# mozendr/FHE-SPEAR

Hardware: AMD Instinct MI355X
Metric: BSGS matvecs/sec at d=2048,N=16384,L0=36; sec/RWKV-block at 1/2/4/8 GPU (higher is better)
Workload: dtype u64

## Files before the change

fhe-spear_amd/csrc/fhs_kernels.hip:

```cpp
#include "fhs_kernels.h"
typedef unsigned long long u64x2_t __attribute__((ext_vector_type(2)));
#ifndef FHS_MODUP_STORE_AUX
#define FHS_MODUP_STORE_AUX 2
#endif
#ifndef FHS_KSIP_UNROLL
#define FHS_KSIP_UNROLL 4
#endif
#include "fhs_ntt.h"
#include "fhs_buffer.h"

#include <atomic>
#include <cstdio>
#include <cstdlib>
#include <cstring>
#include <vector>
#include <algorithm>

#define FHS_INNER_WAVES 16
#define FHS_INNER_VEC 2
#ifndef FHS_MODUPH_CH
#define FHS_MODUPH_CH 2
#endif
#ifndef FHS_MODUPH_RL
#define FHS_MODUPH_RL 3
// ... 1488 lines not shown
                          const KTimer* tm, unsigned* zflag = nullptr) {
    FHS_TMARK(tm, KID_KS_INTT, 1, st);
    if (ks_intt_half<LOGN>(l * U))
        hipLaunchKernelGGL((k_ks_intt_h<LOGN>), dim3(l * U), dim3((1 << LOGN) / 32), 0, st, T, uniq, b.acoef, l, U);
    else
        hipLaunchKernelGGL((k_ks_intt<LOGN>), dim3(l * U), dim3((1 << LOGN) / 16), 0, st, T, uniq, b.acoef, l, U);
    launch_centered(T, b.acoef, b.vcnt, l, U, st, zflag);
    FHS_TMARK(tm, KID_KS_INTT, 0, st);
}
template <int LOGN>
static void ks_modup_stage(const DevTables& T, const u64* const* uniq, int U, int l, const KsBufs& b, hipStream_t st,
                           const KTimer* tm) {
    FHS_TMARK(tm, KID_MODUP, 1, st);
    launch_modup<LOGN>(T, uniq, b.acoef, b.vcnt, b.ext, l, U, st);
    FHS_TMARK(tm, KID_MODUP, 0, st);
}
static void ks_ip_stage(const DevTables& T, const KsItem* it, const u64* const* uniq, int R, int l, const KsBufs& b,
                        hipStream_t st, const KTimer* tm) {
    FHS_TMARK(tm, KID_KS_IP, 1, st);
    hipLaunchKernelGGL(k_ks_ip, dim3(xcd_grid(l + T.P, R * (T.N >> 8))), dim3(256), 0, st, T, it, uniq, b.ext, b.acc, l, R,
                       0);
    FHS_TMARK(tm, KID_KS_IP, 0, st);
}
static void giant_ip_stage(const DevTables& T, const KsItem* it, const u64* const* uniq, int R, int l, const KsBufs& b,
                           hipStream_t st, const KTimer* tm) {
    const int NB = T.N >> 8;
    FHS_TMARK(tm, KID_KS_IP, 1, st);
    hipLaunchKernelGGL(k_ks_ip, dim3(T.P * R * NB), dim3(256), 0, st, T, it, uniq, b.ext, b.acc, l, R, l);
    hipLaunchKernelGGL(k_ks_ip_sum, dim3(xcd_grid(l, NB)), dim3(256), 0, st, T, it, uniq, b.ext, b.acc, l, R);
    FHS_TMARK(tm, KID_KS_IP, 0, st);
}
template <int LOGN>
static void ks_special_intt_stage(const DevTables& T, int R, int l, const KsBufs& b, hipStream_t st, const KTimer* tm) {
    FHS_TMARK(tm, KID_SPECIAL_INTT, 1, st);
    FHS_NTT_LAUNCH(k_ks_special_intt, T.P * 2 * R, dim3(T.P, 2, R), st, T, b.acc, b.ycoef, l, R);
    FHS_TMARK(tm, KID_SPECIAL_INTT, 0, st);
}
template <int LOGN>
static hipError_t ks_moddown_stage(const DevTables& T, const KsItem* it, int R, int l, const KsBufs& b, hipStream_t st,
                                   const KTimer* tm) {
    FHS_TMARK(tm, KID_MODDOWN, 1, st);
    void (*k)(DevTables, const KsItem*, const u64*, const u64*, int, int);
    int nwg = l * 2 * R, threads = (1 << LOGN) / 32;
    const bool xform = ks_uses_half(LOGN) && T.md_xform;
    if (!ks_uses_half(LOGN)) {
        k = k_moddown<LOGN>;
        threads = (1 << LOGN) / 16;
    } else if (xform && T.conv_b59 && LOGN == 15 && nwg < FHS_SPLIT_MAX_WG) {
        k = k_moddown_h<LOGN, true, true, true>;
        nwg *= 2;
    } else if (xform) {
        k = T.conv_b59 ? k_moddown_h<LOGN, true, true> : k_moddown_h<LOGN, true>;
    } else {
        k = T.all_b59 ? k_moddown_h<LOGN, false, true> : k_moddown_h<LOGN, false>;
    }
    if (xform)
        hipLaunchKernelGGL(k_special_x, dim3((T.N + 255) / 256, 2 * R), dim3(256), 0, st, T, b.ycoef, 2 * R);
    hipLaunchKernelGGL(k, dim3(nwg), dim3(threads), 0, st, T, it, b.acc, b.ycoef, l, R);
    FHS_TMARK(tm, KID_MODDOWN, 0, st);
    return hipGetLastError();
}

static hipError_t upload_items(const KsItem* items, int R, const u64* const* uniq, int U, void* dev, const Stager& sg,
                               const KsItem** it_dev, const u64* const** uniq_dev) {
    static thread_local std::vector<unsigned char> buf;
    buf.resize(sizeof(KsItem) * R + sizeof(u64*) * U);
    memcpy(buf.data(), items, sizeof(KsItem) * R);
    memcpy(buf.data() + sizeof(KsItem) * R, uniq, sizeof(u64*) * U);
    hipError_t e = sg.h2d(sg.user, dev, buf.data(), buf.size());
    *it_dev = reinterpret_cast<const KsItem*>(dev);
    *uniq_dev = reinterpret_cast<const u64* const*>(static_cast<unsigned char*>(dev) + sizeof(KsItem) * R);
    return e;
}

__global__ void k_seal_mask(DevTables T, u64 elt, u64* out) {
    const int N = T.N, i = blockIdx.x * blockDim.x + threadIdx.x;
    if (i >= N) return;
    const u64 j = ((u64)i * elt) & (2 * (u64)N - 1);
    const u64 v = j >> T.logN;
    const size_t k = j & (N - 1);
    for (int t = 0; t < T.K; ++t) out[(size_t)t * N + k] = v;
}
__global__ void __launch_bounds__(256) k_seal_corr(DevTables T, const u64* key, const u64* akey, const u64* M,
                                                    int l, u64* out) {
    const int N = T.N, K = T.K, E = l + T.P;
    const int n = blockIdx.x * blockDim.x + threadIdx.x, t = blockIdx.y;
    if (n >= N || t >= E) return;
    const int pt = t < l ? t : T.L0 + (t - l);
    const RedU RD = redu(PK(T, pt));
    const u64 p = RD.q;
    const unsigned qb = 64 - __clzll(p);
    const u64* seeds = key + (size_t)T.dnum * K * N;
    const u64 cx = seeded_ctr_mix(pt, n);
    u128 s0 = {0, 0}, s1 = {0, 0};
    for (int j = 0; j < l; ++j) {
        if (j == t) continue;
        const u64 qj = reduce128(PK(T, j).q, 0, RD);
        const size_t kx = ((size_t)j * K + pt) * N + n;
        const u64 a = akey ? akey[kx] : seeded_uniform_x(seeds[j] + cx, p, qb);
        mac128(s0, key[kx], qj);
        mac128(s1, a, qj);
        if ((j & 7) == 7) {
            s0 = u128{reduce128(s0.lo, s0.hi, RD), 0};
            s1 = u128{reduce128(s1.lo, s1.hi, RD), 0};
        }
    }
    const u64 m = M[(size_t)pt * N + n];
    const u64 r0 = reduce128(s0.lo, s0.hi, RD), r1 = reduce128(s1.lo, s1.hi, RD);
    out[(size_t)t * N + n] = reduce128(r0 * m, __umul64hi(r0, m), RD);
    out[((size_t)E + t) * N + n] = reduce128(r1 * m, __umul64hi(r1, m), RD);
}
hipError_t launch_seal_corr(const DevTables& T, const u64* key, const u64* akey, u64 elt, int l, u64* mask_scratch,
                            u64* out, hipStream_t st) {
    if (T.P != 1 || l < 1 || l > T.L0 || !key || !out || !mask_scratch) return hipErrorInvalidValue;
    hipLaunchKernelGGL(k_seal_mask, dim3((T.N + 255) / 256), dim3(256), 0, st, T, elt, mask_scratch);
    hipError_t e = launch_ntt_fwd(T, mask_scratch, T.K, T.L0, 1, 0, st);
    if (e != hipSuccess) return e;
    hipLaunchKernelGGL(k_seal_corr, dim3((T.N + 255) / 256, l + T.P), dim3(256), 0, st, T, key, akey, mask_scratch,
                       l, out);
    return hipGetLastError();
}

hipError_t launch_keyswitch(const DevTables& T, const KsItem* items_host, int R, const u64* const* uniq_host, int U,
                            int l, u64* ws, size_t ws_bytes, void* items_dev, const Stager& sg, hipStream_t st,
                            const KTimer* tm, SealHoist* sh) {
    if (keyswitch_workspace_bytes(T, R, U, l) > ws_bytes) return hipErrorInvalidValue;
    const KsItem* it;
    const u64* const* uq;
    std::vector<KsItem> sitems;
    std::vector<const u64*> suniq;
    bool hoist = T.ks_seal && sh && U < R;
    for (int r = 0; hoist && r < R; ++r) hoist = items_host[r].elt == 1 || items_host[r].corr;
    if (hoist) {
        hipError_t e = upload_items(items_host, R, uniq_host, U, items_dev, sg, &it, &uq);
        if (e == hipSuccess) e = hipMemsetAsync(sh->zflag_dev, 0, sizeof(unsigned), st);
        if (e != hipSuccess) return e;
        const KsBufs b = ks_carve(T, ws, R, U, l);
        FHS_DISPATCH_LOGN(T.logN, ks_intt_stage<LOGN>(T, uq, U, l, b, st, tm, sh->zflag_dev));
        e = hipMemcpyAsync(sh->zflag_host, sh->zflag_dev, sizeof(unsigned), hipMemcpyDeviceToHost, st);
        if (e == hipSuccess) e = hipStreamSynchronize(st);
        if (e != hipSuccess) return e;
        if (*(volatile unsigned*)sh->zflag_host) {
            ++sh->fallback;
            return launch_keyswitch(T, items_host, R, uniq_host, U, l, ws, ws_bytes, items_dev, sg, st, tm, nullptr);
        }
        ++sh->hoisted;
        FHS_DISPATCH_LOGN(T.logN, {
            ks_modup_stage<LOGN>(T, uq, U, l, b, st, tm);
            ks_ip_stage(T, it, uq, R, l, b, st, tm);
            ks_special_intt_stage<LOGN>(T, R, l, b, st, tm);
            e = ks_moddown_stage<LOGN>(T, it, R, l, b, st, tm);
        });
        if (e != hipSuccess) return e;
        return hipGetLastError();
    }
    if (T.ks_seal) {
        sitems.assign(items_host, items_host + R);
        suniq.resize(R);
        u64* perm = ws + ks_core_bytes(T, R, R, l) / 8;
        seal_rewrite(T, sitems.data(), R, suniq.data(), l, perm);
        hipError_t pe = seal_permute(T, items_host, R, l, perm, st);
        if (pe != hipSuccess) return pe;
        items_host = sitems.data();
        uniq_host = suniq.data();
        U = R;
    }
    hipError_t e = upload_items(items_host, R, uniq_host, U, items_dev, sg, &it, &uq);
    if (e != hipSuccess) return e;
    hipError_t me = hipSuccess;
    const KsBufs b = ks_carve(T, ws, R, U, l);
    FHS_DISPATCH_LOGN(T.logN, {
        ks_intt_stage<LOGN>(T, uq, U, l, b, st, tm);
        ks_modup_stage<LOGN>(T, uq, U, l, b, st, tm);
        ks_ip_stage(T, it, uq, R, l, b, st, tm);
        ks_special_intt_stage<LOGN>(T, R, l, b, st, tm);
        me = ks_moddown_stage<LOGN>(T, it, R, l, b, st, tm);
    });
    if (me != hipSuccess) return me;
    return hipGetLastError();
}

template <int VEC, int TL = 0>
__device__ __forceinline__ void ld_diag(const u64* limb, int voff, int soff, u64* out) {
    const __amdgpu_buffer_rsrc_t r = brsrc(limb, 0x7ffffff0);
    if constexpr (TL > 0) {
        static_assert(VEC == 2, "compact diagonals: two coefficients per lane");
        out[0] = out[1] = __builtin_bit_cast(u64, __builtin_amdgcn_raw_buffer_load_b64(r, voff, soff, kBufNT));
    } else if constexpr (VEC == 2) {
        const auto t = __builtin_amdgcn_raw_buffer_load_b128(r, voff, soff, kBufNT);
        out[0] = ((u64)t[1] << 32) | t[0];
        out[1] = ((u64)t[3] << 32) | t[2];
    } else {
        out[0] = __builtin_bit_cast(u64, __builtin_amdgcn_raw_buffer_load_b64(r, voff, soff, kBufNT));
    }
}
template <int VEC, int WAVES, int FOLD, bool ACC, int TL = 0>
__global__ void __launch_bounds__(64 * WAVES) k_bsgs_inner(DevTables T, const u64* const* __restrict__ baby,
                                                    const u64* const* __restrict__ pts, int G, int Gw, int g0, int g1,
                                                    int D, int l, u64* __restrict__ inner) {
    extern __shared__ __attribute__((aligned(16))) u64 sb[];
    constexpr int W = 64 * VEC;
    const int N = T.N;
    const int i = blockIdx.y, n0 = blockIdx.x * W, tid = threadIdx.x, lane = tid & 63;
    const int wave = __builtin_amdgcn_readfirstlane(tid >> 6);
    const size_t S = (size_t)l * N;
    const size_t off = (size_t)i * N + n0 + lane * VEC;
    const size_t dlimb = (size_t)i * (N >> TL);
    const int dvoff = ((lane * VEC) >> TL) * 8, dsoff = (n0 >> TL) * 8;
    u64 p[8][VEC];
    const int gcur = g0 + wave;
    auto full_batches = [&](int g) { return g < g1 ? max(0, min(Gw, D - g * G)) / 8 : 0; };
    int gf = gcur;
    while (gf < g1 && full_batches(gf) == 0) gf += WAVES;
    if (gf < g1) {
        const u64* const* pg0 = pts + (size_t)gf * G;
#pragma unroll
        for (int u = 0; u < 8; ++u) ld_diag<VEC, TL>(pg0[u] + dlimb, dvoff, dsoff, p[u]);
    }
    for (int idx = tid; idx < Gw * 2 * W; idx += 64 * WAVES) {
        const int b = idx / (2 * W), comp = (idx / W) & 1, c = idx % W;
        sb[idx] = pack30(baby[b][comp * S + (size_t)i * N + n0 + c]);
    }
    __syncthreads();
    const RedU R = redu(PK(T, i));
    for (int g = gcur; g < g1; g += WAVES) {
        const int bmax = min(Gw, D - g * G);
        if (bmax <= 0) continue;
        u128 c0[VEC], c1[VEC];
        Acc3 a0[VEC], a1[VEC];
#pragma unroll
        for (int v = 0; v < VEC; ++v) {
            c0[v] = c1[v] = u128{0, 0};
            a0[v] = a1[v] = Acc3{0, 0, 0};
        }
        const u64* const* pg = pts + (size_t)g * G;
        const int nb = bmax / 8;
        int gn = g + WAVES;
        while (gn < g1 && full_batches(gn) == 0) gn += WAVES;
        int b = 0;
        for (int bi = 0; bi < nb; ++bi, b += 8) {
            constexpr bool ROLL = FOLD == 16;
            if (!ROLL && bi > 0) {
#pragma unroll
                for (int u = 0; u < 8; ++u) ld_diag<VEC, TL>(pg[b + u] + dlimb, dvoff, dsoff, p[u]);
            }
            const u64* const* nxt = ROLL && bi + 1 < nb ? pg + b + 8 : nullptr;
#pragma unroll
            for (int h = 0; h < 8; h += 4) {
#pragma unroll
                for (int u = h; u < h + 4; ++u)
#pragma unroll
                    for (int v = 0; v < VEC; ++v) {
                        const Split30 y = split30(p[u][v]);
                        acc3_mac(a0[v], unpack30(sb[((b + u) * 2 + 0) * W + lane * VEC + v]), y);
                        acc3_mac(a1[v], unpack30(sb[((b + u) * 2 + 1) * W + lane * VEC + v]), y);
                    }
                if (h == 4 && (FOLD == 8 || (b & 15) == 8)) {
#pragma unroll
                    for (int v = 0; v < VEC; ++v) {
                        acc3_fold(c0[v], a0[v]);
                        acc3_fold(c1[v], a1[v]);
                    }
                }
                if (nxt) {
#pragma unroll
                    for (int u = h; u < h + 4; ++u) ld_diag<VEC, TL>(nxt[u] + dlimb, dvoff, dsoff, p[u]);
                }
            }
        }
        for (; b < bmax; ++b) {
            u64 q1[VEC];
            ld_diag<VEC, TL>(pg[b] + dlimb, dvoff, dsoff, q1);
#pragma unroll
            for (int v = 0; v < VEC; ++v) {
                const Split30 y = split30(q1[v]);
                acc3_mac(a0[v], unpack30(sb[(b * 2 + 0) * W + lane * VEC + v]), y);
                acc3_mac(a1[v], unpack30(sb[(b * 2 + 1) * W + lane * VEC + v]), y);
            }
        }
#pragma unroll
        for (int v = 0; v < VEC; ++v) {
            acc3_fold(c0[v], a0[v]);
            acc3_fold(c1[v], a1[v]);
        }
#pragma unroll
        for (int v = 0; v < VEC; ++v) {
            u64* o0 = inner + (size_t)g * 2 * S + off + v;
            u64 r0 = reduce128(c0[v].lo, c0[v].hi, R), r1 = reduce128(c1[v].lo, c1[v].hi, R);
            if constexpr (ACC) {
                r0 = addmod(r0, o0[0], R.q);
                r1 = addmod(r1, o0[S], R.q);
            }
            o0[0] = r0;
            o0[S] = r1;
        }
        if (gn < g1) {
            const u64* const* pgn = pts + (size_t)gn * G;
#pragma unroll
            for (int u = 0; u < 8; ++u) ld_diag<VEC, TL>(pgn[u] + dlimb, dvoff, dsoff, p[u]);
        }
    }
}

#ifndef FHS_GSUM_ICH
#define FHS_GSUM_ICH 4
#endif
__global__ void __launch_bounds__(256) k_giant_sum(DevTables T, const u64* bpart, const u64* ycoef, const u64* inner0,
                                                   u64* base, u64* convsum, int l, int R) {
    const int N = T.N, P_ = T.P, E = l + P_;
    const int n = blockIdx.x * blockDim.x + threadIdx.x, comp = blockIdx.y;
    if (n >= N) return;
    const int i0 = blockIdx.z * FHS_GSUM_ICH, i1 = min(i0 + FHS_GSUM_ICH, l);
    const size_t S = (size_t)l * N;
    constexpr int PMAX = 8;
    u64 ylo[PMAX], yhi[PMAX];
#pragma unroll
    for (int k = 0; k < PMAX; ++k) ylo[k] = yhi[k] = 0;
    for (int r = 0; r < R; ++r) {
        const u64* y = ycoef + ((size_t)r * 2 + comp) * P_ * N + n;
#pragma unroll
        for (int k = 0; k < PMAX; ++k) {
            if (k < P_) {
                const u64 v = y[(size_t)k * N];
                ylo[k] += v;
                yhi[k] += ylo[k] < v;
            }
        }
    }
    for (int i = i0; i < i1; ++i) {
        const PrimeK& P = PK(T, i);
        const u64 q = P.q;
        u128 cs = {0, 0};
#pragma unroll
        for (int k = 0; k < PMAX; ++k)
            if (k < P_) mac128(cs, reduce128(ylo[k], yhi[k], P), T.md_hat[(size_t)k * T.L0 + i]);
        if (T.ks_seal) {
            u128 h = {0, 0};
            mac128(h, (u64)R, T.md_pinv[3 * T.L0 + i]);
            const u64 rh = reduce128(h.lo, h.hi, P);
            cs.lo = reduce128(cs.lo, cs.hi, P);
            cs.hi = 0;
            cs.lo = submod(cs.lo, rh, q);
        }
        u64 cv = reduce128(cs.lo, cs.hi, P);
        const size_t idx = (size_t)comp * S + (size_t)i * N + n;
        const u64 bv = addmod(bpart[((size_t)comp * E + i) * N + n], inner0[idx], q);
        convsum[idx] = cv;
        base[idx] = bv;
    }
}
template <int LOGN, bool H = ntt_half<LOGN>()>
__global__ void __launch_bounds__((ntt_threads<LOGN, H>())) k_giant_final(DevTables T, const u64* base, const u64* convsum,
                                                                     u64* out, int l) {
    constexpr int N = 1 << LOGN;
    __shared__ __attribute__((aligned(16))) u64 lds[ntt_lds_words<LOGN, H>()];
    const int i = blockIdx.x, comp = blockIdx.y;
    const PrimeK& P = PK(T, i);
    const RedU RU = redu(P);
    const size_t off = ((size_t)comp * l + i) * N;
    const u64 pinv = T.md_pinv[2 * i], pinv_s = T.md_pinv[2 * i + 1], q = RU.q;
    fwd_limb<LOGN, FHS_NTT_RL, H>(lds, threadIdx.x, T.tw_fwd + (size_t)i * N * 2, RU,
                               [&](int e) { return convsum[off + e]; },
                               [&](int e, u64 v) { out[off + e] = submod(base[off + e], shoup(v, pinv, pinv_s, q), q); });
}

size_t bsgs_workspace_bytes(const DevTables& T, int R, int l) {
    return keyswitch_workspace_bytes(T, R, R, l) + 8 * (size_t)T.N * 4 * l;
}

template <class Each>
static hipError_t lds_opt_in(std::atomic<bool>& done, size_t bytes, Each each) {
    if (done.load(std::memory_order_acquire)) return hipSuccess;
    hipError_t e = hipSuccess;
    each([&](const void* k) {
        if (k && e == hipSuccess) e = hipFuncSetAttribute(k, hipFuncAttributeMaxDynamicSharedMemorySize, (int)bytes);
    });
    if (e == hipSuccess) done.store(true, std::memory_order_release);
    return e;
}

constexpr int kInnerWindow = 64;
typedef void (*InnerFn)(DevTables, const u64* const*, const u64* const*, int, int, int, int, int, int, u64*);
template <int VEC, int WAVES, int FOLD, int TL>
static InnerFn inner_kernel_acc(bool acc) {
    return acc ? k_bsgs_inner<VEC, WAVES, FOLD, true, TL> : k_bsgs_inner<VEC, WAVES, FOLD, false, TL>;
}
template <int VEC, int WAVES>
static InnerFn inner_kernel(bool fold16, bool acc, int ptl) {
    if (!fold16) return ptl == 0 ? inner_kernel_acc<VEC, WAVES, 8, 0>(acc) : nullptr;
    switch (ptl) {
        case 0: return inner_kernel_acc<VEC, WAVES, 16, 0>(acc);
        case 1: return inner_kernel_acc<VEC, WAVES, 16, 1>(acc);
        case 2: return inner_kernel_acc<VEC, WAVES, 16, 2>(acc);
        case 3: return inner_kernel_acc<VEC, WAVES, 16, 3>(acc);
    }
    return nullptr;
}
template <int VEC, int WAVES>
static hipError_t launch_inner_t(const DevTables& T, const u64* const* baby, const u64* const* pts, int G, int g0,
                                 int g1, int D, int l, u64* inner, hipStream_t st, int ptl) {
    constexpr int W = 64 * VEC;
    static std::atomic<bool> opted{false};
    hipError_t e = lds_opt_in(opted, (size_t)kInnerWindow * 2 * W * 8, [](auto f) {
        for (int fold16 = 0; fold16 < 2; ++fold16)
            for (int acc = 0; acc < 2; ++acc)
                for (int tl = 0; tl <= 3; ++tl)
                    f(reinterpret_cast<const void*>(inner_kernel<VEC, WAVES>(fold16, acc, tl)));
    });
    if (e != hipSuccess) return e;
    if (ptl < 0 || ptl > 3 || (ptl > 0 && (T.max_qbits > 59 || VEC != 2))) return hipErrorInvalidValue;
    for (int b0 = 0; b0 < G; b0 += kInnerWindow) {
        const int Gw = std::min(kInnerWindow, G - b0), Dw = D - b0;
        const size_t lds = (size_t)Gw * 2 * W * 8;
        const dim3 grid(T.N / W, l), block(64 * WAVES);
        const InnerFn k = inner_kernel<VEC, WAVES>(T.max_qbits <= 59, b0 > 0, ptl);
        hipLaunchKernelGGL(k, grid, block, lds, st, T, baby + b0, pts + b0, G, Gw, g0, g1, Dw, l, inner);
        e = hipGetLastError();
        if (e != hipSuccess) return e;
    }
    return hipSuccess;
}

hipError_t launch_bsgs_inner(const DevTables& T, const u64* const* baby_dev, const u64* const* pts_dev, int G, int g0,
                             int g1, int D, int l, u64* inner, hipStream_t st, int ptl) {
    if (T.N % 128 || G < 1) return hipErrorInvalidValue;
    return launch_inner_t<FHS_INNER_VEC, FHS_INNER_WAVES>(T, baby_dev, pts_dev, G, g0, g1, D, l, inner, st, ptl);
}

#define FHS_DOT_WAVES 8
#define FHS_DOT_VEC 2
constexpr int kDotBatch = 4;
template <int VEC, int WAVES, int FOLD, bool ACC>
__global__ void __launch_bounds__(64 * WAVES) k_dot_tensor(DevTables T, const u64* const* __restrict__ q,
                                                          const u64* const* __restrict__ db, int J, int Jw, int C, int l,
                                                          u64* __restrict__ out) {
    extern __shared__ __attribute__((aligned(16))) u64 sb[];
    constexpr int W = 64 * VEC;
    const int N = T.N;
    const int i = blockIdx.y, n0 = blockIdx.x * W, tid = threadIdx.x, lane = tid & 63;
    const int wave = __builtin_amdgcn_readfirstlane(tid >> 6);
    const size_t S = (size_t)l * N;
    const size_t limb = (size_t)i * N;
    const int dvoff = lane * VEC * 8, dsoff = n0 * 8;
    u64 p[kDotBatch][2][VEC];
    auto load_term = [&](const u64* ct, u64 (*dst)[VEC]) {
        ld_diag<VEC>(ct + limb, dvoff, dsoff, dst[0]);
        ld_diag<VEC>(ct + S + limb, dvoff, dsoff, dst[1]);
    };
    const int nb = Jw / kDotBatch;
    if (wave < C && nb > 0) {
        const u64* const* d0 = db + (size_t)wave * J;
#pragma unroll
        for (int u = 0; u < kDotBatch; ++u) load_term(d0[u], p[u]);
    }
    for (int idx = tid; idx < Jw * 2 * W; idx += 64 * WAVES) {
        const int j = idx / (2 * W), comp = (idx / W) & 1, c = idx % W;
        sb[idx] = pack30(q[j][comp * S + limb + n0 + c]);
    }
    __syncthreads();
    const RedU R = redu(PK(T, i));
    for (int c = wave; c < C; c += WAVES) {
        Dot3 s[VEC];
#pragma unroll
        for (int v = 0; v < VEC; ++v) dot3_clear(s[v]);
        const u64* const* dc = db + (size_t)c * J;
        int j = 0;
        for (int bi = 0; bi < nb; ++bi, j += kDotBatch) {
            const u64* const* nxt = bi + 1 < nb ? dc + j + kDotBatch : nullptr;
#pragma unroll
            for (int u = 0; u < kDotBatch; ++u) {
#pragma unroll
                for (int v = 0; v < VEC; ++v)
                    dot3_term<FOLD>(s[v], j + u, unpack30(sb[((j + u) * 2 + 0) * W + lane * VEC + v]),
                                    unpack30(sb[((j + u) * 2 + 1) * W + lane * VEC + v]), split30(p[u][0][v]),
                                    split30(p[u][1][v]));
                if (nxt) load_term(nxt[u], p[u]);
            }
        }
        for (; j < Jw; ++j) {
            u64 t[2][VEC];
            load_term(dc[j], t);
#pragma unroll
            for (int v = 0; v < VEC; ++v)
                dot3_term<FOLD>(s[v], j, unpack30(sb[(j * 2 + 0) * W + lane * VEC + v]),
                                unpack30(sb[(j * 2 + 1) * W + lane * VEC + v]), split30(t[0][v]), split30(t[1][v]));
        }
        u64* o = out + (size_t)c * 3 * S + limb + n0 + lane * VEC;
#pragma unroll
        for (int v = 0; v < VEC; ++v) {
            u64 prev[3], r[3];
            if constexpr (ACC) {
                prev[0] = o[v];
                prev[1] = o[S + v];
                prev[2] = o[2 * S + v];
            }
            dot3_finish(s[v], R, ACC ? prev : nullptr, r);
            o[v] = r[0];
            o[S + v] = r[1];
            o[2 * S + v] = r[2];
        }
        if (c + WAVES < C && nb > 0) {
            const u64* const* dn = db + (size_t)(c + WAVES) * J;
#pragma unroll
            for (int u = 0; u < kDotBatch; ++u) load_term(dn[u], p[u]);
        }
    }
}
typedef void (*DotFn)(DevTables, const u64* const*, const u64* const*, int, int, int, int, u64*);
template <int VEC, int WAVES>
static DotFn dot_kernel(bool fold16, bool acc) {
    if (fold16) return acc ? k_dot_tensor<VEC, WAVES, 16, true> : k_dot_tensor<VEC, WAVES, 16, false>;
    return acc ? k_dot_tensor<VEC, WAVES, 8, true> : k_dot_tensor<VEC, WAVES, 8, false>;
}
template <int VEC, int WAVES>
static hipError_t launch_dot_t(const DevTables& T, const u64* const* q, const u64* const* db, int J, int C, int l, u64* out,
                               hipStream_t st) {
    constexpr int W = 64 * VEC;
    static std::atomic<bool> opted{false};
    hipError_t e = lds_opt_in(opted, (size_t)kDotWindowMax * 2 * W * 8, [](auto f) {
        for (int fold16 = 0; fold16 < 2; ++fold16)
            for (int acc = 0; acc < 2; ++acc) f(reinterpret_cast<const void*>(dot_kernel<VEC, WAVES>(fold16, acc)));
    });
    if (e != hipSuccess) return e;
    for (int j0 = 0; j0 < J; j0 += kDotWindowMax) {
        const int Jw = std::min(kDotWindowMax, J - j0);
        const size_t lds = (size_t)Jw * 2 * W * 8;
        const dim3 grid(T.N / W, l), block(64 * WAVES);
        const DotFn k = dot_kernel<VEC, WAVES>(T.max_qbits <= 59, j0 > 0);
        hipLaunchKernelGGL(k, grid, block, lds, st, T, q + j0, db + j0, J, Jw, C, l, out);
        e = hipGetLastError();
        if (e != hipSuccess) return e;
    }
    return hipSuccess;
}
hipError_t launch_dot_tensor(const DevTables& T, const u64* const* q_dev, const u64* const* db_dev, int J, int C, int l,
                             u64* out3, hipStream_t st, const KTimer* tm) {
    if (T.N % (64 * FHS_DOT_VEC) || J < 1 || C < 1) return hipErrorInvalidValue;
    FHS_TMARK(tm, KID_DOT_TENSOR, 1, st);
    const hipError_t e = launch_dot_t<FHS_DOT_VEC, FHS_DOT_WAVES>(T, q_dev, db_dev, J, C, l, out3, st);
    FHS_TMARK(tm, KID_DOT_TENSOR, 0, st);
    return e;
}

hipError_t launch_bsgs(const DevTables& T, const u64* const* baby_dev, const u64* const* pts_dev, int G, int B, int D,
                       int l, const u64* const* keys_host, const u64* const* akeys_host, const u64* giant_elts, u64* inner,
                       u64* out, u64* ws, size_t ws_bytes, void* items_dev, const Stager& sg, hipStream_t st,
                       const KTimer* tm, int ptl) {
    const int R = B - 1;
    const size_t N = T.N, S = (size_t)l * N;
    if (T.N % 128 || G < 1 || R > 512) return hipErrorInvalidValue;
    if (R > 0 && bsgs_workspace_bytes(T, R, l) > ws_bytes) return hipErrorInvalidValue;
    KsItem items[512];
    const u64* uniq[512];
    for (int r = 0; r < R; ++r) {
        const int g = r + 1;
        const u64* ct = inner + (size_t)g * 2 * S;
        u64 elt = 1;
        if (giant_elts) elt = giant_elts[g];
        else
            for (int s2 = 0; s2 < g * G; ++s2) elt = (elt * 5) & (2 * N - 1);
        items[r] = KsItem{ct + S, ct, nullptr, keys_host[g], nullptr, nullptr, elt, (u64)r,
                          akeys_host ? akeys_host[g] : nullptr};
        uniq[r] = ct + S;
    }
    std::vector<KsItem> seal_orig;
    u64* seal_perm = ws + ks_core_bytes(T, R, R, l) / 8;
    if (T.ks_seal && R > 0) {
        seal_orig.assign(items, items + R);
        seal_rewrite(T, items, R, uniq, l, seal_perm);
    }
    const KsItem* it = nullptr;
    const u64* const* uq = nullptr;
    if (R > 0) {
        hipError_t e = upload_items(items, R, uniq, R, items_dev, sg, &it, &uq);
        if (e != hipSuccess) return e;
    }
    hipError_t he = hipSuccess;
    if (pts_dev) {
        FHS_TMARK(tm, KID_BSGS_INNER, 1, st);
        he = launch_inner_t<FHS_INNER_VEC, FHS_INNER_WAVES>(T, baby_dev, pts_dev, G, 0, B, D, l, inner, st, ptl);
        FHS_TMARK(tm, KID_BSGS_INNER, 0, st);
        if (he != hipSuccess) return he;
    }
    if (R <= 0) return hipMemcpyAsync(out, inner, 8 * 2 * S, hipMemcpyDeviceToDevice, st);
    if (!seal_orig.empty()) {
        he = seal_permute(T, seal_orig.data(), R, l, seal_perm, st);
        if (he != hipSuccess) return he;
    }
    u64* base = ws + keyswitch_workspace_bytes(T, R, R, l) / 8;
    u64* convsum = base + 2 * S;
    FHS_DISPATCH_LOGN(T.logN, {
        const KsBufs b = ks_carve(T, ws, R, R, l);
        ks_intt_stage<LOGN>(T, uq, R, l, b, st, tm);
        ks_modup_stage<LOGN>(T, uq, R, l, b, st, tm);
        giant_ip_stage(T, it, uq, R, l, b, st, tm);
        ks_special_intt_stage<LOGN>(T, R, l, b, st, tm);
        FHS_TMARK(tm, KID_GIANT_SUM, 1, st);
        hipLaunchKernelGGL(k_giant_sum, dim3((T.N + 255) / 256, 2, (l + FHS_GSUM_ICH - 1) / FHS_GSUM_ICH), dim3(256), 0,
                           st, T, b.acc, b.ycoef, inner, base, convsum, l, R);
        FHS_TMARK(tm, KID_GIANT_SUM, 0, st);
        FHS_TMARK(tm, KID_GIANT_FINAL, 1, st);
        FHS_NTT_LAUNCH(k_giant_final, l * 2, dim3(l, 2), st, T, base, convsum, out, l);
        FHS_TMARK(tm, KID_GIANT_FINAL, 0, st);
    });
    return hipGetLastError();
}



__device__ __forceinline__ u64 rnd_testdata(u64 key, u64 ctr) { return sm64(key ^ sm64(ctr ^ 0xD1B54A32D192ED03ULL)); }

__global__ void k_sample(DevTables T, int mode, PrfKey K, u64 sid, u64* out, int l, u64 sid_step, u64* const* outs) {
    const int N = T.N;
    const size_t S = (size_t)l * N;
    sid += blockIdx.y * sid_step;
    out = outs ? outs[blockIdx.y] : out + blockIdx.y * S;
    for (size_t idx = blockIdx.x * (size_t)blockDim.x + threadIdx.x; idx < S; idx += (size_t)gridDim.x * blockDim.x) {
        const int i = (int)(idx / N), n = (int)(idx % N);
        const PrimeK& P = PK(T, i);
        u64 v;
        if (mode == SAMPLE_UNIFORM) {
            u64 hi, lo;
            prf128(K, sid, (uint32_t)idx, hi, lo);
            v = reduce128(lo, hi, P);
        } else if (mode == SAMPLE_SEEDED) {
            v = seeded_uniform_x(sid + seeded_ctr_mix(i, n), P.q, 64 - __clzll(P.q));
        } else if (mode == SAMPLE_TESTDATA) {
            const u64 ctr = 2 * ((u64)i * N + n);
            v = reduce128(rnd_testdata(sid, ctr + 1), rnd_testdata(sid, ctr), P);
        } else {
            u64 r, unused;
            prf128(K, sid, (uint32_t)n, r, unused);
            long long s;
            if (mode == SAMPLE_TERNARY) {
                const u64 t = r % 3;
                s = t == 2 ? -1 : (long long)t;
            } else {
                s = (long long)__popcll(r & 0x1FFFFFULL) - (long long)__popcll((r >> 21) & 0x1FFFFFULL);
            }
            v = s >= 0 ? (u64)s : P.q - (u64)(-s);
        }
        out[idx] = v;
    }
}
hipError_t launch_sample(const DevTables& T, int mode, const PrfKey& K, u64 sid, u64* out, int l, hipStream_t st,
                         int npoly, u64 sid_step, u64* const* outs_dev) {
    if (npoly < 1) return hipSuccess;
    const int g1 = eltwise_grid((size_t)l * T.N) / npoly, gx = g1 > 0 ? g1 : 1;
    hipLaunchKernelGGL(k_sample, dim3(gx, npoly), dim3(256), 0, st, T, mode, K, sid, out, l, sid_step, outs_dev);
    return hipGetLastError();
}

__global__ void k_swk(DevTables T, u64* b_out, const u64* a, const u64* e, const u64* s, const u64* snew, int j) {
    const int N = T.N, K = T.K;
    const size_t S = (size_t)K * N;
    for (size_t idx = blockIdx.x * (size_t)blockDim.x + threadIdx.x; idx < S; idx += (size_t)gridDim.x * blockDim.x) {
        const int i = (int)(idx / N);
        const PrimeK& P = PK(T, i);
        u64 v = submod(e[idx], mulmod(a[idx], s[idx], P), P.q);
        if (i < T.L0 && i / T.P == j) {
            const u64 pm = T.md_pinv[2 * T.L0 + i];
            v = addmod(v, mulmod(pm, snew[idx], P), P.q);
        }
        b_out[idx] = v;
    }
}
hipError_t launch_switch_key_assemble(const DevTables& T, u64* b_out, const u64* a, const u64* e_ntt, const u64* s_ntt,
                                      const u64* snew_ntt, int digit, hipStream_t st) {
    hipLaunchKernelGGL(k_swk, dim3(eltwise_grid((size_t)T.K * T.N)), dim3(256), 0, st, T, b_out, a, e_ntt, s_ntt,
                       snew_ntt, digit);
    return hipGetLastError();
}

__global__ void k_encrypt(DevTables T, int mode, u64* c0, u64* c1, const u64* s_or_pk0, const u64* pk1, const u64* u,
                          const u64* e0, const u64* e1, const u64* pt, int l) {
    const int N = T.N;
    const size_t S = (size_t)l * N;
    for (size_t idx = blockIdx.x * (size_t)blockDim.x + threadIdx.x; idx < S; idx += (size_t)gridDim.x * blockDim.x) {
        const int i = (int)(idx / N);
        const PrimeK& P = PK(T, i);
        const u64 q = P.q;
        const u64 m = pt ? pt[idx] : 0;
        if (mode == 0) {
            c0[idx] = addmod(submod(e0[idx], mulmod(c1[idx], s_or_pk0[idx], P), q), m, q);
        } else {
            c0[idx] = addmod(addmod(mulmod(u[idx], s_or_pk0[idx], P), e0[idx], q), m, q);
            c1[idx] = addmod(mulmod(u[idx], pk1[idx], P), e1[idx], q);
        }
    }
}
__global__ void k_sample_small(int mode, PrfKey K, u64 sid, u64 sid_step, int N, signed char* out) {
    sid += blockIdx.y * sid_step;
    out += (size_t)blockIdx.y * N;
    for (int n = blockIdx.x * blockDim.x + threadIdx.x; n < N; n += gridDim.x * blockDim.x) {
        u64 r, unused;
        prf128(K, sid, (uint32_t)n, r, unused);
        int v;
        if (mode == SAMPLE_TERNARY) {
            const u64 t = r % 3;
            v = t == 2 ? -1 : (int)t;
        } else {
            v = __popcll(r & 0x1FFFFFULL) - __popcll((r >> 21) & 0x1FFFFFULL);
        }
        out[n] = (signed char)v;
    }
}
template <int LOGN>
__global__ void __launch_bounds__(ntt_threads<LOGN>()) k_ntt_fwd_small(DevTables T, const signed char* small, u64* out,
                                                                      int limbs) {
    constexpr int N = 1 << LOGN;
    __shared__ __attribute__((aligned(16))) u64 lds[ntt_lds_words<LOGN>()];
    const int b = blockIdx.x;
    const RedU R = redu(PK(T, b));
    const signed char* sm = small + (size_t)blockIdx.y * N;
    u64* p = out + ((size_t)blockIdx.y * limbs + b) * N;
    const u64 q = R.q;
    fwd_limb<LOGN, FHS_NTT_RL>(lds, threadIdx.x, T.tw_fwd + (size_t)b * N * 2, R,
                               [&](int e) { const int v = sm[e]; return v >= 0 ? (u64)v : q - (u64)(-v); },
                               [&](int e, u64 v) { p[e] = v; });
}
struct DblMod {
    const PrimeK* P;
    const u64* pow2;
    u64 q, mask;
    unsigned b, d;
    bool fold1;
};
__device__ __forceinline__ DblMod dbl_mod_of(const DevTables& T, int i) {
    const PrimeK& P = PK(T, i);
    const u64 pm = P.pm, q = P.q;
    const unsigned b = (unsigned)(pm & 127), d = (unsigned)((pm >> 8) & 0xFFFFFFFFu);
    const bool fold1 = b != 0 && ((u64)d << (64 - b)) + (1ull << b) < 2 * q;
    return DblMod{&P, T.pow2 + (size_t)i * 1088, q, b ? (1ull << b) - 1 : 0, b, d, fold1};
}
__device__ __forceinline__ u64 dbl_mod(const DblMod& M, double v) {
    const bool neg = v < 0;
    const double a = neg ? -v : v;
    u64 r;
    if (a < 9.2e18) {
        const u64 x = (u64)a;
        r = M.fold1 ? csub((x & M.mask) + mul32w((uint32_t)(x >> M.b), M.d), M.q) : reduce64(x, *M.P);
    } else {
        const PrimeK& P = *M.P;
        const u64 bits = (u64)__double_as_longlong(a);
        const int ex = (int)((bits >> 52) & 0x7FF) - 1075;
        const u64 mant = (bits & ((1ULL << 52) - 1)) | (1ULL << 52);
        r = mulmod(reduce64(mant, P), M.pow2[ex], P);
    }
    return (neg && r) ? M.q - r : r;
}
__device__ __forceinline__ u64 dbl_mod(const DevTables& T, double d, int i) { return dbl_mod(dbl_mod_of(T, i), d); }
__device__ __forceinline__ RedU enc_lazy(RedU R, const DblMod& M) {
    if (M.fold1 && R.q < (1ull << 59)) R.lazy = true;
    return R;
}
template <int LOGN>
__global__ void __launch_bounds__(ntt_threads<LOGN>()) k_ntt_fwd_msg_err(DevTables T, const double* coef,
                                                                        const signed char* small, u64* out, int limbs) {
    constexpr int N = 1 << LOGN;
    __shared__ __attribute__((aligned(16))) u64 lds[ntt_lds_words<LOGN>()];
    const int b = blockIdx.x;
    const RedU R = redu(PK(T, b));
    const double* cf = coef + (size_t)blockIdx.y * N;
    const signed char* sm = small + (size_t)blockIdx.y * N;
    u64* p = out + ((size_t)blockIdx.y * limbs + b) * N;
    const u64 q = R.q;
    const DblMod M = dbl_mod_of(T, b);
    fwd_limb<LOGN, FHS_NTT_RL>(lds, threadIdx.x, T.tw_fwd + (size_t)b * N * 2, enc_lazy(R, M),
                               [&](int e) {
                                   const int v = sm[e];
                                   return dbl_mod(M, cf[e]) + (v >= 0 ? (u64)v : q - (u64)(-v));
                               },
                               [&](int e, u64 v) { p[e] = v; });
}
__global__ void k_encrypt_sym(DevTables T, PrfKey K, u64 sid, u64 sid_step, u64* const* cts, const u64* s,
                              const u64* eb, const u64* const* pts, int l) {
    const int N = T.N;
    const size_t S = (size_t)l * N;
    sid += blockIdx.y * sid_step;
    u64* c0 = cts[blockIdx.y];
    u64* c1 = c0 + S;
    const u64* e = eb + blockIdx.y * S;
    const u64* m = pts ? pts[blockIdx.y] : nullptr;
    for (size_t idx = blockIdx.x * (size_t)blockDim.x + threadIdx.x; idx < S; idx += (size_t)gridDim.x * blockDim.x) {
        const PrimeK& P = PK(T, (int)(idx / N));
        const u64 q = P.q;
        u64 hi, lo;
        prf128(K, sid, (uint32_t)idx, hi, lo);
        const u64 a = reduce128(lo, hi, P);
        c1[idx] = a;
        const u64 c = submod(e[idx], mulmod(a, s[idx], P), q);
        c0[idx] = m ? addmod(c, m[idx], q) : c;
    }
}
hipError_t launch_encrypt_sym_batch(const DevTables& T, const PrfKey& K, u64 sid_mask, u64 sid_err, u64 sid_step,
                                    u64* const* cts_dev, const u64* s, const u64* const* pts_dev, int count, int l,
                                    signed char* small, u64* eb, hipStream_t st, const double* coef) {
    if (count <= 0) return hipSuccess;
    hipLaunchKernelGGL(k_sample_small, dim3((T.N + 255) / 256, count), dim3(256), 0, st, (int)SAMPLE_CBD, K, sid_err,
                       sid_step, T.N, small);
    FHS_DISPATCH_LOGN(T.logN, {
        if (coef)
            hipLaunchKernelGGL((k_ntt_fwd_msg_err<LOGN>), dim3(l, count), dim3(ntt_threads<LOGN>()), 0, st, T, coef,
                               static_cast<const signed char*>(small), eb, l);
        else
            hipLaunchKernelGGL((k_ntt_fwd_small<LOGN>), dim3(l, count), dim3(ntt_threads<LOGN>()), 0, st, T,
                               static_cast<const signed char*>(small), eb, l);
    });
    const int g1 = eltwise_grid((size_t)l * T.N) / count, gx = g1 > 0 ? g1 : 1;
    hipLaunchKernelGGL(k_encrypt_sym, dim3(gx, count), dim3(256), 0, st, T, K, sid_mask, sid_step, cts_dev, s,
                       static_cast<const u64*>(eb), pts_dev, l);
    return hipGetLastError();
}
hipError_t launch_encrypt_combine(const DevTables& T, int mode, u64* c0, u64* c1, const u64* s_or_pk0, const u64* pk1,
                                  const u64* u_ntt, const u64* e0, const u64* e1, const u64* pt, int l, hipStream_t st) {
    hipLaunchKernelGGL(k_encrypt, dim3(eltwise_grid((size_t)l * T.N)), dim3(256), 0, st, T, mode, c0, c1, s_or_pk0,
                       pk1, u_ntt, e0, e1, pt, l);
    return hipGetLastError();
}

__global__ void k_decrypt(DevTables T, const u64* ct, int ncomp, const u64* s, u64* out, int l) {
    const int N = T.N;
    const size_t S = (size_t)l * N;
    for (size_t idx = blockIdx.x * (size_t)blockDim.x + threadIdx.x; idx < S; idx += (size_t)gridDim.x * blockDim.x) {
        const int i = (int)(idx / N);
        const PrimeK& P = PK(T, i);
        const u64 sv = s[idx];
        u64 v = ct[idx], sp = sv;
        for (int k = 1; k < ncomp; ++k) {
            v = addmod(v, mulmod(ct[k * S + idx], sp, P), P.q);
            sp = mulmod(sp, sv, P);
        }
        out[idx] = v;
    }
}
__global__ void k_decrypt_many(DevTables T, const u64* const* cts, int ncomp, const u64* s, u64* out, size_t out_stride,
                               int l) {
    const int N = T.N;
    const size_t S = (size_t)l * N;
    const u64* ct = cts[blockIdx.y];
    u64* o = out + blockIdx.y * out_stride;
    for (size_t idx = blockIdx.x * (size_t)blockDim.x + threadIdx.x; idx < S; idx += (size_t)gridDim.x * blockDim.x) {
        const PrimeK& P = PK(T, (int)(idx / N));
        const u64 sv = s[idx];
        u64 v = ct[idx], sp = sv;
        for (int k = 1; k < ncomp; ++k) {
            v = addmod(v, mulmod(ct[k * S + idx], sp, P), P.q);
            sp = mulmod(sp, sv, P);
        }
        o[idx] = v;
    }
}
hipError_t launch_decrypt_many(const DevTables& T, const u64* const* cts_dev, int count, int ncomp, const u64* s, u64* out,
                               size_t out_stride, int l, hipStream_t st) {
    if (count <= 0) return hipSuccess;
    const int g1 = eltwise_grid((size_t)l * T.N) / count, gx = g1 > 0 ? g1 : 1;
    hipLaunchKernelGGL(k_decrypt_many, dim3(gx, count), dim3(256), 0, st, T, cts_dev, ncomp, s, out, out_stride, l);
    return hipGetLastError();
}
hipError_t launch_decrypt(const DevTables& T, const u64* ct, int ncomp, const u64* s, u64* out, int l, hipStream_t st) {
    hipLaunchKernelGGL(k_decrypt, dim3(eltwise_grid((size_t)l * T.N)), dim3(256), 0, st, T, ct, ncomp, s, out, l);
    return hipGetLastError();
}


__global__ void k_encode_reduce(DevTables T, const double* coef, int count, u64* out, int l) {
    const int N = T.N;
    const size_t total = (size_t)count * l * N;
    for (size_t idx = blockIdx.x * (size_t)blockDim.x + threadIdx.x; idx < total;
         idx += (size_t)gridDim.x * blockDim.x) {
        const int n = (int)(idx % N);
        const size_t rest = idx / N;
        const int i = (int)(rest % l);
        const size_t v = rest / l;
        out[idx] = dbl_mod(T, coef[v * N + n], i);
    }
}

template <class BF>
__device__ __forceinline__ void fft_dit_stages(double2* a, int tid, int TH, int n_pts, int log_pts, const double2* W,
                                               int logh, BF bf) {
    int s = 0;
    for (; s + 1 < log_pts; s += 2) {
        const int half = 1 << s;
        for (int g = tid; g < n_pts / 4; g += TH) {
            const int k = g & (half - 1);
            const int i0 = ((g >> s) << (s + 2)) + k;
            double2 x0 = a[i0], x1 = a[i0 + half], x2 = a[i0 + 2 * half], x3 = a[i0 + 3 * half];
            const double2 w = W[(size_t)k << (logh - 1 - s)];
            bf(x0, x1, w);
            bf(x2, x3, w);
            bf(x0, x2, W[(size_t)k << (logh - 2 - s)]);
            bf(x1, x3, W[(size_t)(k + half) << (logh - 2 - s)]);
            a[i0] = x0;
            a[i0 + half] = x1;
            a[i0 + 2 * half] = x2;
            a[i0 + 3 * half] = x3;
        }
        __syncthreads();
    }
    if (s < log_pts) {
        const int half = 1 << s;
// ... 591 lines not shown
```

Baseline: 158.2.

## Split giant-sum reduction over R across waves and reduce partial sums in LDS

Rewrites k_giant_sum so that each block handles 64 coefficients with FHS_GSUM_RS waves. The waves divide the R ycoef rows among themselves, and their partial 128-bit sums are combined through shared memory. Each wave then processes a strided subset of primes. Previously every block along the prime-chunk axis re-read all R*P ycoef rows, and the summation over R ran serially per thread. The kernel is now templated on P so loops fully unroll, with loads unrolled and bpart/inner0 loads hoisted. The trade-offs are a block-level sync, a 32-bit carry accumulator, and a hard limit of P at most 8.

Result: no change. 160.1, median of 6 (+1.2%).

```diff
diff --git a/fhe-spear_amd/csrc/fhs_kernels.hip b/fhe-spear_amd/csrc/fhs_kernels.hip
--- a/fhe-spear_amd/csrc/fhs_kernels.hip
+++ b/fhe-spear_amd/csrc/fhs_kernels.hip
@@ -1814,38 +1814,68 @@
     }
 }
 
-#ifndef FHS_GSUM_ICH
-#define FHS_GSUM_ICH 4
+#ifndef FHS_GSUM_RS
+#define FHS_GSUM_RS 8
 #endif
-__global__ void __launch_bounds__(256) k_giant_sum(DevTables T, const u64* bpart, const u64* ycoef, const u64* inner0,
-                                                   u64* base, u64* convsum, int l, int R) {
-    const int N = T.N, P_ = T.P, E = l + P_;
-    const int n = blockIdx.x * blockDim.x + threadIdx.x, comp = blockIdx.y;
-    if (n >= N) return;
-    const int i0 = blockIdx.z * FHS_GSUM_ICH, i1 = min(i0 + FHS_GSUM_ICH, l);
+template <int PC>
+__global__ void __launch_bounds__(64 * FHS_GSUM_RS) k_giant_sum(DevTables T, const u64* __restrict__ bpart,
+                                                                const u64* __restrict__ ycoef,
+                                                                const u64* __restrict__ inner0, u64* __restrict__ base,
+                                                                u64* __restrict__ convsum, int l, int R) {
+    constexpr int RS = FHS_GSUM_RS, UR = (8 + PC - 1) / PC;
+    __shared__ u64 slo[RS][PC][64];
+    __shared__ uint32_t shi[RS][PC][64];
+    const int N = T.N, E = l + PC;
+    const int lane = threadIdx.x & 63, s = __builtin_amdgcn_readfirstlane(threadIdx.x >> 6);
+    const int n = blockIdx.x * 64 + lane, comp = blockIdx.y;
     const size_t S = (size_t)l * N;
-    constexpr int PMAX = 8;
-    u64 ylo[PMAX], yhi[PMAX];
-#pragma unroll
-    for (int k = 0; k < PMAX; ++k) ylo[k] = yhi[k] = 0;
-    for (int r = 0; r < R; ++r) {
-        const u64* y = ycoef + ((size_t)r * 2 + comp) * P_ * N + n;
-#pragma unroll
-        for (int k = 0; k < PMAX; ++k) {
-            if (k < P_) {
-                const u64 v = y[(size_t)k * N];
-                ylo[k] += v;
-                yhi[k] += ylo[k] < v;
+    u64 ylo[PC];
+    uint32_t yhi[PC];
+#pragma unroll
+    for (int k = 0; k < PC; ++k) ylo[k] = yhi[k] = 0;
+    const u64* y0 = ycoef + (size_t)comp * PC * N + n;
+    for (int r0 = s; r0 < R; r0 += RS * UR) {
+        u64 v[UR][PC];
+#pragma unroll
+        for (int u = 0; u < UR; ++u) {
+            const int r = r0 + u * RS;
+#pragma unroll
+            for (int k = 0; k < PC; ++k) v[u][k] = r < R ? y0[((size_t)r * 2 * PC + k) * N] : 0;
+        }
+#pragma unroll
+        for (int u = 0; u < UR; ++u)
+#pragma unroll
+            for (int k = 0; k < PC; ++k) {
+                ylo[k] += v[u][k];
+                yhi[k] += ylo[k] < v[u][k];
             }
-        }
-    }
-    for (int i = i0; i < i1; ++i) {
+    }
+#pragma unroll
+    for (int k = 0; k < PC; ++k) {
+        slo[s][k][lane] = ylo[k];
+        shi[s][k][lane] = yhi[k];
+    }
+    __syncthreads();
+    u64 tlo[PC], thi[PC];
+#pragma unroll
+    for (int k = 0; k < PC; ++k) {
+        tlo[k] = thi[k] = 0;
+#pragma unroll
+        for (int s2 = 0; s2 < RS; ++s2) {
+            const u64 v = slo[s2][k][lane];
+            tlo[k] += v;
+            thi[k] += shi[s2][k][lane] + (tlo[k] < v);
+        }
+    }
+#pragma unroll 2
+    for (int i = s; i < l; i += RS) {
         const PrimeK& P = PK(T, i);
         const u64 q = P.q;
+        const size_t idx = (size_t)comp * S + (size_t)i * N + n;
+        const u64 bp = bpart[((size_t)comp * E + i) * N + n], in0 = inner0[idx];
         u128 cs = {0, 0};
 #pragma unroll
-        for (int k = 0; k < PMAX; ++k)
-            if (k < P_) mac128(cs, reduce128(ylo[k], yhi[k], P), T.md_hat[(size_t)k * T.L0 + i]);
+        for (int k = 0; k < PC; ++k) mac128(cs, reduce128(tlo[k], thi[k], P), T.md_hat[(size_t)k * T.L0 + i]);
         if (T.ks_seal) {
             u128 h = {0, 0};
             mac128(h, (u64)R, T.md_pinv[3 * T.L0 + i]);
@@ -1854,12 +1884,25 @@
             cs.hi = 0;
             cs.lo = submod(cs.lo, rh, q);
         }
-        u64 cv = reduce128(cs.lo, cs.hi, P);
-        const size_t idx = (size_t)comp * S + (size_t)i * N + n;
-        const u64 bv = addmod(bpart[((size_t)comp * E + i) * N + n], inner0[idx], q);
-        convsum[idx] = cv;
-        base[idx] = bv;
-    }
+        convsum[idx] = reduce128(cs.lo, cs.hi, P);
+        base[idx] = addmod(bp, in0, q);
+    }
+}
+static void launch_giant_sum(const DevTables& T, const u64* bpart, const u64* ycoef, const u64* inner0, u64* base,
+                             u64* convsum, int l, int R, hipStream_t st) {
+    void (*k)(DevTables, const u64*, const u64*, const u64*, u64*, u64*, int, int) = nullptr;
+    switch (T.P) {
+        case 1: k = k_giant_sum<1>; break;
+        case 2: k = k_giant_sum<2>; break;
+        case 3: k = k_giant_sum<3>; break;
+        case 4: k = k_giant_sum<4>; break;
+        case 5: k = k_giant_sum<5>; break;
+        case 6: k = k_giant_sum<6>; break;
+        case 7: k = k_giant_sum<7>; break;
+        case 8: k = k_giant_sum<8>; break;
+        default: return;
+    }
+    hipLaunchKernelGGL(k, dim3(T.N / 64, 2), dim3(64 * FHS_GSUM_RS), 0, st, T, bpart, ycoef, inner0, base, convsum, l, R);
 }
 template <int LOGN, bool H = ntt_half<LOGN>()>
 __global__ void __launch_bounds__((ntt_threads<LOGN, H>())) k_giant_final(DevTables T, const u64* base, const u64* convsum,
@@ -2060,7 +2103,7 @@
                        const KTimer* tm, int ptl) {
     const int R = B - 1;
     const size_t N = T.N, S = (size_t)l * N;
-    if (T.N % 128 || G < 1 || R > 512) return hipErrorInvalidValue;
+    if (T.N % 128 || G < 1 || R > 512 || T.P < 1 || T.P > 8) return hipErrorInvalidValue;
     if (R > 0 && bsgs_workspace_bytes(T, R, l) > ws_bytes) return hipErrorInvalidValue;
     KsItem items[512];
     const u64* uniq[512];
@@ -2108,8 +2151,7 @@
         giant_ip_stage(T, it, uq, R, l, b, st, tm);
         ks_special_intt_stage<LOGN>(T, R, l, b, st, tm);
         FHS_TMARK(tm, KID_GIANT_SUM, 1, st);
-        hipLaunchKernelGGL(k_giant_sum, dim3((T.N + 255) / 256, 2, (l + FHS_GSUM_ICH - 1) / FHS_GSUM_ICH), dim3(256), 0,
-                           st, T, b.acc, b.ycoef, inner, base, convsum, l, R);
+        launch_giant_sum(T, b.acc, b.ycoef, inner, base, convsum, l, R, st);
         FHS_TMARK(tm, KID_GIANT_SUM, 0, st);
         FHS_TMARK(tm, KID_GIANT_FINAL, 1, st);
         FHS_NTT_LAUNCH(k_giant_final, l * 2, dim3(l, 2), st, T, base, convsum, out, l);
```
